# crockwell/far

Measured on AMD Instinct MI355X. Metric: image-pairs/sec (match+solve+regress) at 640x480, higher is better.
Workload: dtype f32

## Files before the change

### far_amd/_lib.py

```python
import ctypes
import os

from . import flags

_HERE = os.path.dirname(os.path.abspath(__file__))
LIB_PATH = flags.value('FAR_HIP_LIB') or os.path.join(_HERE, 'lib', 'libfar_hip.so')

c_p = ctypes.c_void_p
c_i = ctypes.c_int
c_f = ctypes.c_float
c_d = ctypes.c_double
c_sz = ctypes.c_size_t
c_l = ctypes.c_long
c_u32 = ctypes.c_uint32

SIGNATURES = {
    'far_abi_version': (c_i, []),
    'far_last_hip_error': (c_i, []),
    'far_set_tuning': (c_i, [c_i, c_i]),
    'far_mfma_probe_f16': (c_i, [c_i, c_i, c_i, c_p, c_p, c_p]),
    'far_dual_softmax_workspace_bytes': (c_sz, [c_i, c_i, c_i]),
    'far_dual_softmax_stats_f32': (c_i, [c_p, c_p, c_i, c_i, c_i, c_i, c_f, c_f, c_f, c_p, c_p, c_p, c_p, c_p, c_p]),
    'far_coarse_match_f32': (c_i, [c_p, c_p, c_i, c_i, c_i, c_i, c_f, c_f, c_i, c_i, c_i, c_i, c_i, c_f,
                                   c_p, c_p, c_p, c_p, c_p, c_p, c_p, c_p, c_p, c_p, c_p, c_p, c_p, c_p, c_p, c_p]),
    'far_coarse_match_bf16_workspace_bytes': (c_sz, [c_i, c_i, c_i, c_i]),
    'far_coarse_match_bf16': (c_i, [c_p, c_p, c_i, c_i, c_i, c_i, c_f, c_f, c_i, c_i, c_i, c_i, c_i, c_f,
                                    c_p, c_p, c_p, c_p, c_p, c_p, c_p, c_p, c_p, c_p, c_p, c_p, c_p, c_p, c_p, c_p]),
    'far_coarse_match_f16s_workspace_bytes': (c_sz, [c_i, c_i, c_i, c_i]),
    'far_coarse_match_f16s': (c_i, [c_p, c_p, c_i, c_i, c_i, c_i, c_f, c_f, c_i, c_i, c_i, c_i, c_i, c_f,
                                    c_p, c_p, c_p, c_p, c_p, c_p, c_p, c_p, c_p, c_p, c_p, c_p, c_p, c_p, c_p, c_p, c_p]),
    'far_conf_matrix_f16s': (c_i, [c_p, c_p, c_i, c_i, c_i, c_i, c_f, c_p, c_p, c_i, c_p, c_p, c_p, c_p, c_p]),
    'far_coarse_match_sinkhorn_f16s_workspace_bytes': (c_sz, [c_i, c_i, c_i, c_i]),
    'far_coarse_match_sinkhorn_f16s': (c_i, [c_p, c_p, c_i, c_i, c_i, c_i, c_p, c_i, c_i, c_f, c_i, c_i, c_i, c_i, c_i, c_f,
                                             c_p, c_p, c_p, c_p, c_p, c_p, c_p, c_p, c_p, c_p, c_p, c_p, c_p, c_p, c_p, c_p,
                                             c_p, c_p, c_p]),
    'far_coarse_train_workspace_bytes': (c_sz, [c_i, c_i, c_i, c_i]),
    'far_coarse_pos_conf_f16s': (c_i, [c_p, c_p, c_i, c_i, c_i, c_i, c_f, c_p, c_p, c_p, c_i, c_p, c_p, c_p, c_p]),
    'far_coarse_pos_conf_bwd_f16': (c_i, [c_p, c_p, c_i, c_i, c_i, c_i, c_f, c_p, c_p, c_p, c_i, c_p, c_p, c_p, c_p, c_p]),
    'far_sinkhorn_pos_conf_workspace_bytes': (c_sz, [c_i, c_i, c_i, c_i, c_i]),
    'far_sinkhorn_pos_conf_f16s': (c_i, [c_p, c_p, c_i, c_i, c_i, c_i, c_p, c_i, c_p, c_p, c_p, c_p, c_p, c_i, c_p, c_p, c_p,
                                         c_p, c_p, c_p]),
    'far_sinkhorn_pos_conf_bwd_f16': (c_i, [c_p, c_p, c_i, c_i, c_i, c_i, c_p, c_i, c_p, c_p, c_p, c_p, c_p, c_i, c_p, c_p, c_p,
                                            c_p, c_p, c_p, c_p, c_p]),
    'far_emm_pv_f32': (c_i, [c_p, c_p, c_p, c_p, c_i, c_i, c_i, c_f, c_p, c_p, c_p, c_p]),
    'far_fine_gather_f32': (c_i, [c_p, c_l, c_l, c_l, c_l, c_i, c_i, c_i, c_p, c_p, c_i, c_i, c_i, c_i, c_p, c_p]),
    'far_fine_scatter_f32': (c_i, [c_p, c_l, c_l, c_l, c_l, c_i, c_i, c_i, c_p, c_p, c_i, c_i, c_i, c_i, c_p, c_p]),
    'far_fine_scatter_det_f32': (c_i, [c_p, c_l, c_l, c_l, c_l, c_i, c_i, c_i, c_p, c_p, c_i, c_i, c_i, c_i, c_i, c_i, c_p, c_p]),
    'far_fine_expect_f32': (c_i, [c_p, c_p, c_i, c_i, c_i, c_p, c_f, c_p, c_p, c_p, c_p, c_p]),
    'far_linear_attention_workspace_bytes': (c_sz, [c_i, c_i, c_i, c_i]),
    'far_linear_attention_f32': (c_i, [c_p, c_p, c_p, c_i, c_i, c_i, c_i, c_i, c_p, c_p, c_f, c_p, c_p, c_p]),
    'far_linear_attention_apply_f32': (c_i, [c_p, c_p, c_i, c_i, c_i, c_i, c_p, c_f, c_p, c_p]),
    'far_full_attention_workspace_bytes': (c_sz, [c_i, c_i, c_i, c_i, c_i]),
    'far_full_attention_f16s': (c_i, [c_p, c_p, c_p, c_i, c_i, c_i, c_i, c_i, c_p, c_p, c_i, c_p, c_p, c_p, c_p]),
    'far_full_attention_train_f16s': (c_i, [c_p, c_p, c_p, c_i, c_i, c_i, c_i, c_i, c_p, c_p, c_i, c_p, c_p, c_p, c_p, c_p]),
    'far_full_attention_bwd_workspace_bytes': (c_sz, [c_i, c_i, c_i, c_i, c_i]),
    'far_full_attention_bwd_f16s': (c_i, [c_p, c_p, c_p, c_p, c_p, c_p, c_i, c_i, c_i, c_i, c_i, c_p, c_p, c_i, c_p, c_p, c_p, c_p, c_p, c_p]),
    'far_linear_attention_bwd_workspace_bytes': (c_sz, [c_i, c_i, c_i, c_i, c_i]),
    'far_linear_attention_bwd_f32': (c_i, [c_p, c_p, c_p, c_p, c_i, c_i, c_i, c_i, c_i, c_p, c_p, c_f, c_p, c_p, c_p, c_p, c_p]),
    'far_layernorm_f32': (c_i, [c_p, c_p, c_p, c_p, c_l, c_i, c_f, c_p, c_p]),
    'far_layernorm_bwd_ws_bytes': (c_l, [c_l, c_i]),
    'far_layernorm_bwd_f32': (c_i, [c_p, c_p, c_p, c_l, c_i, c_f, c_p, c_p, c_p, c_p, c_l, c_p]),
    'far_attn_block_packed_bytes': (c_sz, [c_i]),
    'far_attn_block_f16s': (c_i, [c_p, c_p, c_p, c_l, c_i, c_i, c_i, c_i, c_f, c_f, c_f, c_f, c_f, c_p, c_p, c_f, c_p, c_p, c_p]),
    'far_mlp_fused_packed_bytes': (c_sz, [c_i]),
    'far_mlp_fused_f16s': (c_i, [c_p, c_p, c_p, c_l, c_i, c_f, c_f, c_p, c_p, c_f, c_p, c_p, c_p]),
    'far_mlp_fused_f16': (c_i, [c_p, c_p, c_p, c_l, c_i, c_f, c_f, c_p, c_p, c_f, c_p, c_p, c_p]),
    'far_attn_block_f16': (c_i, [c_p, c_p, c_p, c_l, c_i, c_i, c_i, c_i, c_f, c_f, c_f, c_f, c_f, c_p, c_p, c_f, c_p, c_p, c_p]),
    'far_affine_act_f32': (c_i, [c_p, c_p, c_p, c_p, c_l, c_i, c_l, c_i, c_i, c_f, c_p, c_p]),
    'far_upsample2x_add_f32': (c_i, [c_p, c_p, c_i, c_i, c_i, c_i, c_i, c_p, c_p]),
    'far_upsample2x_bwd_f32': (c_i, [c_p, c_i, c_i, c_i, c_i, c_p, c_p]),
    'far_adamw_table_bytes': (c_l, [c_i, c_l]),
    'far_adamw_step_f32': (c_i, [c_p, c_i, c_l] + [ctypes.c_double] * 7 + [c_p]),
    'far_prior_from_pose_f32': (c_i, [c_p, c_p, c_p, c_i, c_p, c_p]),
    'far_bn_train_ws_bytes': (c_l, [c_l, c_i]),
    'far_bn_act_train_fwd_f32': (c_i, [c_p, c_p, c_l, c_i, c_p, c_p, c_f, c_f, c_p, c_p, c_i, c_f, c_p, c_p, c_p, c_l, c_p]),
    'far_bn_train_stats_f32': (c_i, [c_p, c_l, c_i, c_p, c_p, c_f, c_f, c_p, c_p, c_p, c_p, c_p, c_p, c_p, c_l, c_p]),
    'far_bn_train_bwd_f32': (c_i, [c_p, c_p, c_p, c_p, c_p, c_p, c_l, c_i, c_i, c_f, c_p, c_p, c_p, c_p, c_p, c_l, c_p]),
    'far_conv_packed_bytes': (c_sz, [c_i, c_i, c_i, c_i, c_i]),
    'far_conv_pack_f32': (c_i, [c_p, c_i, c_i, c_i, c_i, c_i, c_i, c_p, c_p]),
    'far_weight_scale_f32': (c_i, [c_p, c_l, c_p, c_p]),
    'far_conv_pack_view_f32': (c_i, [c_p, c_l, c_l, c_l, c_i, c_i, c_i, c_i, c_i, c_p, c_p, c_p]),
    'far_enc_layer_saved_floats': (c_l, [c_p]),
    'far_enc_layer_grads_floats': (c_l, [c_p]),
# ... 126 lines not shown
```

### far_amd/csrc/dual_softmax_f16s.hip

```cpp
#include "k1_f16s.h"
#include <algorithm>

int far_k1_conf_launch(const _Float16* ah, const _Float16* bh, int Z, int L, int S, int Lp, int Sp, float c1, float fill2,
                       const uint8_t* mask0, const uint8_t* mask1, const float2* rowstat, const float* cmax,
                       const float* cinv, float* conf, const int* fix_count, const uint2* fix_list, int slots,
                       int* fix_info_out, hipStream_t stream);

namespace {

constexpr int CAND_SLOTS = 4;

#define FAR_DPP(old, v, ctrl, rowmask) \
    __builtin_bit_cast(float, __builtin_amdgcn_update_dpp(__builtin_bit_cast(int, old), __builtin_bit_cast(int, v), ctrl, rowmask, 0xF, false))
__device__ __forceinline__ float max32_to_upper_row(float v) {
    v = fmaxf(v, FAR_DPP(v, v, 0xB1, 0xF));
    v = fmaxf(v, FAR_DPP(v, v, 0x4E, 0xF));
    v = fmaxf(v, FAR_DPP(v, v, 0x141, 0xF));
    v = fmaxf(v, FAR_DPP(v, v, 0x140, 0xF));
    v = fmaxf(v, FAR_DPP(v, v, 0x142, 0xA));
    return v;
}

template <bool CAND>
__global__ __launch_bounds__(256, 2) void k1_rowstats(const _Float16* __restrict__ ah, const _Float16* __restrict__ al,
// ... 42 lines not shown
        const float resc = __builtin_amdgcn_exp2f(m - mn);
        float t = 0.f;
#pragma unroll
        for (int ct = 0; ct < 2; ++ct)
#pragma unroll
            for (int r = 0; r < 16; ++r) t += __builtin_amdgcn_exp2f(acc[ct][r] - mn);
        sum *= resc;
        comp *= resc;
        const float y = t - comp;
        const float ns = sum + y;
        comp = (ns - sum) - y;
        sum = ns;
        m = mn;
        if (CAND) {
            const float clog = m + __builtin_amdgcn_logf(sum - comp);
            float hot = -1.f;
            const float* tl = reinterpret_cast<const float*>(lds + 2 * TILE_PLANE);
#pragma unroll
            for (int ct = 0; ct < 2; ++ct)
#pragma unroll
                for (int q4 = 0; q4 < 4; ++q4) {
                    const float4 a = *reinterpret_cast<const float4*>(tl + 32 * ct + 8 * q4 + 4 * h);
                    hot = fmaxf(hot, fmaxf(fmaxf(2.0f * acc[ct][4 * q4 + 0] - a.x, 2.0f * acc[ct][4 * q4 + 1] - a.y),
                                           fmaxf(2.0f * acc[ct][4 * q4 + 2] - a.z, 2.0f * acc[ct][4 * q4 + 3] - a.w)));
                }
            if (__builtin_amdgcn_ballot_w64(hot >= clog) != 0ull) {
                uint2* const slots = cand + ((size_t)z * Nr + min(irow, Nr - 1)) * (2 * CAND_SLOTS) + h * CAND_SLOTS;
#pragma unroll 1
                for (int ct = 0; ct < 2; ++ct)
#pragma unroll
                    for (int r = 0; r < 16; ++r) {
                        const int i = jt * KT + 32 * ct + mfma32_row(r, h);
                        const float xv = ct == 0 ? acc[0][r] : acc[1][r];
                        if (2.0f * xv >= tl[32 * ct + mfma32_row(r, h)] + clog && xv > -1.0e8f && i < Nc && irow < Nr) {
                            if (ncand < CAND_SLOTS) slots[ncand] = make_uint2((unsigned)i, __float_as_uint(xv));
                            ++ncand;
                        }
                    }
            }
        }
    }
    if (CAND && irow < Nr) cand_count[((size_t)z * Nr + irow) * 2 + h] = ncand;
    sum -= comp;
    const float mo = shfl_xor_f(m, 32), so = shfl_xor_f(sum, 32);
    const float mn = fmaxf(m, mo);
    const float st = sum * __builtin_amdgcn_exp2f(m - mn) + so * __builtin_amdgcn_exp2f(mo - mn);
    if (h == 0) {
        if (irow < Nr) stat[(size_t)z * Nr + irow] = make_float2(mn, st);
        if (dmax) {
            dmax[(size_t)z * Nrp + irow] = irow < Nr ? mn : HUGE_F;
            dinv[(size_t)z * Nrp + irow] = irow < Nr ? 1.0f / st : 0.f;
        }
        if (dthr) dthr[(size_t)z * Nrp + irow] = irow < Nr ? mn + __builtin_amdgcn_logf(st) - 12.0f : HUGE_F;
    }
}

__global__ __launch_bounds__(256, 2) void k1_screen(const _Float16* __restrict__ ah, const _Float16* __restrict__ bh, int Z, int L, int S,
                                                    int Lp, int Sp, float c1, const float2* __restrict__ rowstat,
                                                    const float* __restrict__ cmax, float thr, const unsigned* __restrict__ nmax,
                                                    uint8_t* __restrict__ tmask) {
    extern __shared__ __attribute__((aligned(16))) unsigned char lds[];
    const int tid = threadIdx.x, wave = tid >> 6, lane = tid & 63, l31 = lane & 31, h = lane >> 5;
    const int nI = Lp / 128;
    int z, Ib;
    tile_coords(nI, Z, z, Ib);
    const int irow = Ib * 128 + 32 * wave + l31;
    f16x8 rh[NS];
#pragma unroll
    for (int s = 0; s < NS; ++s)
        rh[s] = *reinterpret_cast<const f16x8*>(ah + ((size_t)z * Lp + irow) * C + 8 * ((2 * s + h) ^ (irow & 15)));
    const float rmax = irow < L ? rowstat[(size_t)z * L + irow].x : HUGE_F;
    const float c2 = 2.0f * c1;
    const float slack2 = c2 * __builtin_sqrtf(__uint_as_float(nmax[0]) * __uint_as_float(nmax[1])) *
                         (1.0f / 1024.0f * (1.0f + 1.0f / 2048.0f) + 1.0f / 8192.0f);
    const float lim = __builtin_amdgcn_logf(thr) + rmax - slack2;
    const int ntile = (S + KT - 1) / KT;
    for (int jt = 0; jt < ntile; ++jt) {
        __syncthreads();
        {
            const unsigned char* sh = reinterpret_cast<const unsigned char*>(bh + ((size_t)z * Sp + jt * KT) * C) + tid * 16;
#pragma unroll
            for (int j = 0; j < TILE_PLANE / 4096; ++j)
                __builtin_amdgcn_global_load_lds((gptr_t)(sh + j * 4096), (lptr_t)(lds + j * 4096 + wave * 1024), 16, 0, 0);
        }
        asm volatile("s_waitcnt vmcnt(0)" ::: "memory");
        __syncthreads();
        f32x16 acc[2];
#pragma unroll
        for (int ct = 0; ct < 2; ++ct)
#pragma unroll
            for (int r = 0; r < 16; ++r) acc[ct][r] = 0.f;
#pragma unroll
        for (int s = 0; s < NS; ++s)
#pragma unroll
            for (int ct = 0; ct < 2; ++ct) {
                const int row = 32 * ct + l31;
                const f16x8 ch = *reinterpret_cast<const f16x8*>(lds + row * ROWB + (((2 * s + h) ^ (row & 15)) * 16));
                acc[ct] = __builtin_amdgcn_mfma_f32_32x32x16_f16(ch, rh[s], acc[ct], 0, 0, 0);
            }
        float top = -HUGE_F;
#pragma unroll
        for (int ct = 0; ct < 2; ++ct)
#pragma unroll
            for (int q4 = 0; q4 < 4; ++q4) {
                const float4 a = *reinterpret_cast<const float4*>(cmax + (size_t)z * Sp + jt * KT + 32 * ct + 8 * q4 + 4 * h);
                top = fmaxf(top, fmaxf(fmaxf(fmaf(acc[ct][4 * q4 + 0], c2, -a.x), fmaf(acc[ct][4 * q4 + 1], c2, -a.y)),
// ... 49 lines not shown
                const size_t o = (size_t)z * Sp + jt * KT + 32 * ct + 8 * q4 + 4 * h;
                const float4 a = *reinterpret_cast<const float4*>(cmax + o), b = *reinterpret_cast<const float4*>(cinv + o);
                cm[4 * q4 + 0] = a.x; cm[4 * q4 + 1] = a.y; cm[4 * q4 + 2] = a.z; cm[4 * q4 + 3] = a.w;
                ci[4 * q4 + 0] = b.x; ci[4 * q4 + 1] = b.y; ci[4 * q4 + 2] = b.z; ci[4 * q4 + 3] = b.w;
            }
#pragma unroll
            for (int r = 0; r < 16; ++r) {
                const int j = jt * KT + 32 * ct + mfma32_row(r, h);
                float x2 = acc[ct][r] * c2;
                if (masks && j < S && (rmasked || (mask1 && !mask1[(size_t)z * S + j]))) x2 = 2.0f * fill2;
                const float p = __builtin_amdgcn_exp2f((x2 - rst.x) - cm[r]) * rinv * ci[r];
                const bool valid = ivalid && j < S;
                acc[ct][r] = valid ? p : -1.f;
                if (valid && p > bestv) { bestv = p; bestj = j; }
            }
            if (CONF && ivalid) {
#pragma unroll
                for (int q4 = 0; q4 < 4; ++q4) {
                    const int j = jt * KT + 32 * ct + 8 * q4 + 4 * h;
                    float* dst = conf + ((size_t)z * L + irow) * S + j;
                    if (aligned4 && j + 3 < S) {
                        *reinterpret_cast<float4*>(dst) = make_float4(acc[ct][4 * q4], acc[ct][4 * q4 + 1], acc[ct][4 * q4 + 2], acc[ct][4 * q4 + 3]);
                    } else {
#pragma unroll
                        for (int e = 0; e < 4; ++e)
                            if (j + e < S) dst[e] = acc[ct][4 * q4 + e];
                    }
                }
            }
            float tmax = fmaxf(fmaxf(acc[ct][0], acc[ct][1]), fmaxf(acc[ct][2], acc[ct][3]));
#pragma unroll
            for (int r = 4; r < 16; r += 2) tmax = fmaxf(tmax, fmaxf(acc[ct][r], acc[ct][r + 1]));
            if (__builtin_amdgcn_ballot_w64(tmax > thr) != 0ull) {
#pragma unroll
                for (int r = 0; r < 16; ++r)
                    if (acc[ct][r] > thr)
                        atomicMax(colbest + (size_t)z * S + jt * KT + 32 * ct + mfma32_row(r, h), __float_as_uint(acc[ct][r]));
            }
        }
    }
    const float vo = shfl_xor_f(bestv, 32);
    const int jo = shfl_xor_i(bestj, 32);
    if (vo > bestv || (vo == bestv && jo < bestj)) { bestv = vo; bestj = jo; }
    if (h == 0 && ivalid) {
        rowbest_v[(size_t)z * L + irow] = bestv;
        rowbest_j[(size_t)z * L + irow] = bestj;
    }
}

struct Ws16 {
    K1Workspace k;
    _Float16 *ah, *al, *bh, *bl;
    float2* colstat2;
    float *cmax, *cinv;
    float* rthr;
    uint8_t* tmask;
    unsigned* nmax;
    int* fix_count;
    uint2* fix_list;
    size_t bytes;
};
inline Ws16 carve16(void* ws, int Z, int L, int S) {
    Ws16 w;
    w.k = carve(ws, Z, L, S);
    const int Lp = (L + 127) / 128 * 128, Sp = (S + 127) / 128 * 128;
    unsigned char* p = (unsigned char*)ws;
    size_t o = w.k.bytes;
    auto take = [&](size_t n) { unsigned char* r = p ? p + o : nullptr; o += align256(n); return r; };
    w.ah = (_Float16*)take((size_t)Z * Lp * C * 2); w.al = (_Float16*)take((size_t)Z * Lp * C * 2);
    w.bh = (_Float16*)take((size_t)Z * Sp * C * 2); w.bl = (_Float16*)take((size_t)Z * Sp * C * 2);
    w.colstat2 = (float2*)take((size_t)Z * S * 8);
    w.cmax = (float*)take((size_t)Z * Sp * 4); w.cinv = (float*)take((size_t)Z * Sp * 4);
    w.rthr = (float*)take((size_t)Z * Lp * 4);
    w.nmax = (unsigned*)take(2 * sizeof(unsigned));
    w.tmask = (uint8_t*)take((size_t)Z * (Lp / 128) * ((S + KT - 1) / KT) * 4);
    w.fix_count = (int*)take((size_t)Z * S * 2 * sizeof(int));
    w.fix_list = (uint2*)take((size_t)Z * S * 2 * CAND_SLOTS * sizeof(uint2));
    w.bytes = o;
    return w;
}

}

size_t far_k1_fwd_ws_bytes(int Z, int L, int S) { return carve16(nullptr, Z, L, S).bytes; }

static float k1_c1(float temperature) {
    return (float)(1.4426950408889634 / ((double)C * (double)temperature * PRESCALE * PRESCALE));
}

int far_k1_stats_launch(const float* f0, const float* f1, int Z, int L, int S, float temperature, void* ws, int* overflow,
                        hipStream_t stream) {
    const Ws16 w = carve16(ws, Z, L, S);
    const int Lp = (L + 127) / 128 * 128, Sp = (S + 127) / 128 * 128;
    const float c1 = k1_c1(temperature), fill2 = -1e9f * 1.44269504088896341f;
    auto gridp = [](long n) { long b = (n + 255) / 256; return (unsigned)(b < 65536L * 4 ? b : 65536L * 4); };
    hipLaunchKernelGGL(k1_prep, dim3(gridp((long)Z * Lp * 32)), dim3(256), 0, stream, f0, Z, L, Lp, w.ah, w.al, overflow, (unsigned*)nullptr);
    hipLaunchKernelGGL(k1_prep, dim3(gridp((long)Z * Sp * 32)), dim3(256), 0, stream, f1, Z, S, Sp, w.bh, w.bl, overflow, (unsigned*)nullptr);
    const size_t smem_s = 2 * TILE_PLANE + KT * sizeof(float);
    FAR_ONCE_PER_DEVICE(hipFuncSetAttribute((const void*)k1_rowstats<false>, hipFuncAttributeMaxDynamicSharedMemorySize, (int)smem_s));
    hipLaunchKernelGGL(k1_rowstats<false>, dim3((Lp / 128) * Z), dim3(256), smem_s, stream, w.ah, w.al, w.bh, w.bl, Z, L, S, Lp, Sp,
                       c1, fill2, (const uint8_t*)nullptr, (const uint8_t*)nullptr, w.k.rowstat, (float*)nullptr, (float*)nullptr,
                       (float*)nullptr, (const float*)nullptr, (int*)nullptr, (uint2*)nullptr);
    hipLaunchKernelGGL(k1_rowstats<false>, dim3((Sp / 128) * Z), dim3(256), smem_s, stream, w.bh, w.bl, w.ah, w.al, Z, S, L, Sp, Lp,
                       c1, fill2, (const uint8_t*)nullptr, (const uint8_t*)nullptr, w.colstat2, w.cmax, w.cinv, (float*)nullptr,
                       (const float*)nullptr, (int*)nullptr, (uint2*)nullptr);
    return far_check_launch();
}

void far_k1_fwd_views(void* ws, int Z, int L, int S, const _Float16** ah, const _Float16** bh, const float2** rowstat,
                      const float** cmax, const float** cinv, float* c1_out) {
    const Ws16 w = carve16(ws, Z, L, S);
    *ah = w.ah; *bh = w.bh; *rowstat = w.k.rowstat; *cmax = w.cmax; *cinv = w.cinv;
    *c1_out = 0.f;
}

extern "C" {

size_t far_coarse_match_f16s_workspace_bytes(int Z, int L, int S, int Cc) {
    if (Z <= 0 || L <= 0 || S <= 0 || Cc != C) return 0;
    return carve16(nullptr, Z, L, S).bytes;
}

int far_coarse_match_f16s(const float* f0, const float* f1, int Z, int L, int S, int Cc,
                          float temperature, float thr, int border, int h0, int w0, int h1, int w1,
                          float cell_scale, const uint8_t* mask0, const uint8_t* mask1,
                          const int* valid_hw, const float* scale0, const float* scale1,
                          float* conf_out, int64_t* b_ids, int64_t* i_ids, int64_t* j_ids, float* mconf,
                          float* mkpts0_c, float* mkpts1_c, int* counts_out, int* total_out,
                          void* ws, int* overflow, hipStream_t stream) {
    far_clear_errors();
    if (!f0 || !f1 || !ws || !b_ids || !i_ids || !j_ids || !mconf || !mkpts0_c || !mkpts1_c || !total_out)
        return FAR_EINVAL;
    if (Z <= 0 || L <= 0 || S <= 0 || Cc != C || h0 * w0 != L || h1 * w1 != S || (long)Z * (L > S ? L : S) > 0x7ff00000L) return FAR_EINVAL;
    const Ws16 w = carve16(ws, Z, L, S);
    const int Lp = (L + 127) / 128 * 128, Sp = (S + 127) / 128 * 128;
    const float c1 = (float)(1.4426950408889634 / ((double)C * (double)temperature * PRESCALE * PRESCALE));
    const float fill2 = -1e9f * 1.44269504088896341f;
    auto gridp = [](long n) { long b = (n + 255) / 256; return (unsigned)(b < 65536L * 4 ? b : 65536L * 4); };
    const bool screen = !conf_out && !mask0 && !mask1 && far_get_tuning(10) == 0;
    if (screen) hipMemsetAsync(w.nmax, 0, 2 * sizeof(unsigned), stream);
    hipLaunchKernelGGL(k1_prep, dim3(gridp((long)Z * Lp * 32)), dim3(256), 0, stream, f0, Z, L, Lp, w.ah, w.al, overflow, screen ? w.nmax : (unsigned*)nullptr);
    hipLaunchKernelGGL(k1_prep, dim3(gridp((long)Z * Sp * 32)), dim3(256), 0, stream, f1, Z, S, Sp, w.bh, w.bl, overflow, screen ? w.nmax + 1 : (unsigned*)nullptr);
    int* counts = counts_out ? counts_out : w.k.counts;
    hipMemsetAsync(counts, 0, sizeof(int) * Z, stream);
    const size_t smem_s = 2 * TILE_PLANE + KT * sizeof(float), smem_m = 2 * TILE_PLANE + 4 * 64 * sizeof(float);
    FAR_ONCE_PER_DEVICE(
        hipFuncSetAttribute((const void*)k1_rowstats<false>, hipFuncAttributeMaxDynamicSharedMemorySize, (int)smem_s);
        hipFuncSetAttribute((const void*)k1_match<false>, hipFuncAttributeMaxDynamicSharedMemorySize, (int)smem_m);
        hipFuncSetAttribute((const void*)k1_match<true>, hipFuncAttributeMaxDynamicSharedMemorySize, (int)smem_m));
    hipLaunchKernelGGL(k1_rowstats<false>, dim3((Lp / 128) * Z), dim3(256), smem_s, stream, w.ah, w.al, w.bh, w.bl, Z, L, S, Lp, Sp,
                       c1, fill2, mask0, mask1, w.k.rowstat, (float*)nullptr, (float*)nullptr, (float*)nullptr,
                       (const float*)nullptr, (int*)nullptr, (uint2*)nullptr);
    hipLaunchKernelGGL(k1_rowstats<false>, dim3((Sp / 128) * Z), dim3(256), smem_s, stream, w.bh, w.bl, w.ah, w.al, Z, S, L, Sp, Lp,
                       c1, fill2, mask1, mask0, w.colstat2, w.cmax, w.cinv, (float*)nullptr, (const float*)nullptr,
                       (int*)nullptr, (uint2*)nullptr);
    const int nI = Lp / 128;
    hipMemsetAsync(w.k.colbest_part, 0, sizeof(float) * (size_t)Z * S, stream);
    if (screen) {
        FAR_ONCE_PER_DEVICE(hipFuncSetAttribute((const void*)k1_screen, hipFuncAttributeMaxDynamicSharedMemorySize, (int)TILE_PLANE));
        hipLaunchKernelGGL(k1_screen, dim3(nI * Z), dim3(256), TILE_PLANE, stream, w.ah, w.bh, Z, L, S, Lp, Sp, c1, w.k.rowstat, w.cmax, thr,
                           (const unsigned*)w.nmax, w.tmask);
    }
    if (conf_out)
        hipLaunchKernelGGL(k1_match<true>, dim3(nI * Z), dim3(256), smem_m, stream, w.ah, w.al, w.bh, w.bl, Z, L, S, Lp, Sp, c1,
                           fill2, mask0, mask1, w.k.rowstat, w.cmax, w.cinv, conf_out, w.k.rowbest_v, w.k.rowbest_j, reinterpret_cast<unsigned*>(w.k.colbest_part), thr,
                           screen ? (const uint8_t*)w.tmask : (const uint8_t*)nullptr);
    else
        hipLaunchKernelGGL(k1_match<false>, dim3(nI * Z), dim3(256), smem_m, stream, w.ah, w.al, w.bh, w.bl, Z, L, S, Lp, Sp, c1,
                           fill2, mask0, mask1, w.k.rowstat, w.cmax, w.cinv, conf_out, w.k.rowbest_v, w.k.rowbest_j, reinterpret_cast<unsigned*>(w.k.colbest_part), thr,
                           screen ? (const uint8_t*)w.tmask : (const uint8_t*)nullptr);
    hipLaunchKernelGGL(k_finalize, dim3((L + 255) / 256, Z), dim3(256), 0, stream, w.k.rowbest_v, w.k.rowbest_j,
                       w.k.colbest_part, 1, L, S, thr, border, h0, w0, h1, w1, valid_hw, w.k.match_j, counts);
    hipLaunchKernelGGL(k_compact, dim3(Z), dim3(256), 0, stream, w.k.match_j, w.k.rowbest_v, counts, L, w0, w1,
                       cell_scale, scale0, scale1, b_ids, i_ids, j_ids, mconf, mkpts0_c, mkpts1_c, total_out);
    return far_check_launch();
}

int far_conf_matrix_f16s(const float* f0, const float* f1, int Z, int L, int S, int Cc, float temperature,
                         const uint8_t* mask0, const uint8_t* mask1, int stages, float* conf_out, int* fix_info_out,
                         void* ws, int* overflow, hipStream_t stream) {
    far_clear_errors();
    if (!f0 || !f1 || !ws || !conf_out || Z <= 0 || L <= 0 || S <= 0 || Cc != C || !(stages & 3) || (long)Z * (L > S ? L : S) > 0x7ff00000L) return FAR_EINVAL;
    const Ws16 w = carve16(ws, Z, L, S);
    const int Lp = (L + 127) / 128 * 128, Sp = (S + 127) / 128 * 128;
    const float c1 = (float)(1.4426950408889634 / ((double)C * (double)temperature * PRESCALE * PRESCALE));
    const float fill2 = -1e9f * 1.44269504088896341f;
    if (stages & 1) {
        auto gridp = [](long n) { long b = (n + 255) / 256; return (unsigned)(b < 65536L * 4 ? b : 65536L * 4); };
        hipLaunchKernelGGL(k1_prep, dim3(gridp((long)Z * Lp * 32)), dim3(256), 0, stream, f0, Z, L, Lp, w.ah, w.al, overflow, (unsigned*)nullptr);
        hipLaunchKernelGGL(k1_prep, dim3(gridp((long)Z * Sp * 32)), dim3(256), 0, stream, f1, Z, S, Sp, w.bh, w.bl, overflow, (unsigned*)nullptr);
        const size_t smem_s = 2 * TILE_PLANE + KT * sizeof(float);
        FAR_ONCE_PER_DEVICE(
            hipFuncSetAttribute((const void*)k1_rowstats<false>, hipFuncAttributeMaxDynamicSharedMemorySize, (int)smem_s);
            hipFuncSetAttribute((const void*)k1_rowstats<true>, hipFuncAttributeMaxDynamicSharedMemorySize, (int)smem_s));
        hipLaunchKernelGGL(k1_rowstats<false>, dim3((Lp / 128) * Z), dim3(256), smem_s, stream, w.ah, w.al, w.bh, w.bl, Z, L, S, Lp,
                           Sp, c1, fill2, mask0, mask1, w.k.rowstat, (float*)nullptr, (float*)nullptr, w.rthr,
                           (const float*)nullptr, (int*)nullptr, (uint2*)nullptr);
        hipLaunchKernelGGL(k1_rowstats<true>, dim3((Sp / 128) * Z), dim3(256), smem_s, stream, w.bh, w.bl, w.ah, w.al, Z, S, L, Sp,
                           Lp, c1, fill2, mask1, mask0, w.colstat2, w.cmax, w.cinv, (float*)nullptr, (const float*)w.rthr,
                           w.fix_count, w.fix_list);
    }
    if (stages & 2) {
        const int rc = far_k1_conf_launch(w.ah, w.bh, Z, L, S, Lp, Sp, c1, fill2, mask0, mask1, w.k.rowstat, w.cmax, w.cinv,
                                          conf_out, w.fix_count, w.fix_list, CAND_SLOTS, fix_info_out, stream);
        if (rc != FAR_OK) return rc;
    }
    return far_check_launch();
}

}
```

### far_amd/flags.py

```python
import os
from collections import namedtuple

Switch = namedtuple('Switch', 'env module attr off_value neutral scope doc')
SWITCHES = [
    Switch('FAR_NO_WINO', 'far_amd.ops', 'USE_WINO', False, 'parity', 'inference',
           'stride-1 3x3 convolutions on K9 (direct implicit GEMM) instead of K17 (Winograd F(2x2,3x3)); same operator, other summation'),
    Switch('FAR_NO_PAD', 'far_amd.loftr.backbone', 'PAD_CHANNELS', False, 'bitwise', 'inference',
           'the 196-channel backbone maps stored with 196 channels instead of 208 (zero weights for the extra ones: exact zeros)'),
    Switch('FAR_NO_PREFETCH', 'far_amd.loftr.model:LoFTR', 'head_prefetch', False, 'bitwise', 'inference',
           "the head's feature stage computed inside forward_rt_prediction instead of enqueued behind K1"),
    Switch('FAR_NO_SIDE_STREAM', 'far_amd.loftr.model:LoFTR', 'head_side_stream', False, 'bitwise', 'inference',
           "the head's feature stage on the step's own stream behind K1 (rounds 2-5) instead of on a second stream next to K1 and the fine level"),
    Switch('FAR_FPN_STREAM', 'far_amd.loftr.model:LoFTR', 'fpn_side_stream', True, 'bitwise', 'inference',
           "OPT-IN (1 switches it ON; default off): the FPN's fine branch on a side stream next to the coarse transformer and K1 (-0.6 ms per 32 "
           "pairs; off by default because the roofline launch -- K17 208 -> 208 @ 240x320 -- then shares the GPU and its in-step duration "
           "in a kernel trace is no longer its own)"),
    Switch('FAR_NO_GATHER_FUSE', 'far_amd.loftr.stages:FinePreprocess', 'fused_gather', False, 'bitwise', 'inference',
           'FinePreprocess.merge_feat on a materialised window tensor (K3 gather + K9) instead of K9 reading through the match indices'),
    Switch('FAR_NO_KV', 'far_amd.loftr.transformer:LoFTREncoderLayer', 'fused_kv', False, 'parity', 'inference',
           "k, v projections + K5's first half as separate launches instead of K9's k|v epilogue (the K'^T V sum changes order)"),
    Switch('FAR_NO_QAPPLY', 'far_amd.loftr.transformer:LoFTREncoderLayer', 'fused_apply', False, 'parity', 'inference',
           "q projection + K5's second half as separate launches instead of K9's attention-apply epilogue (q no longer stays in split operands)"),
    Switch('FAR_NO_STACK', 'far_amd.loftr.transformer:LocalFeatureTransformer', 'stack_self', False, 'bitwise', 'inference',
           "the two 'self' calls of an encoder layer on the two images separately instead of one call on both"),
    Switch('FAR_NO_BN', 'far_amd.ops', 'USE_HIP_BATCHNORM_TRAIN', False, 'parity', 'training',
           'training-mode BatchNorm on nn.BatchNorm2d + torch activations instead of K19 (tests/test_train_kernels_gpu.py holds K19 to the module)'),
]

ENV_ONLY = {
    'FAR_HIP_LIB': ('load', 'path of another build of libfar_hip.so (tools/ab_build.py: same-box A/B against a git revision); skips the build-id check'),
    'FAR_TUNING': ('load', 'comma-separated key=value pairs handed to far_set_tuning at load time, e.g. FAR_TUNING="10=1,8=1" (keys below)'),
    'FAR_SKIP_ASM_CHECK': ('build', "1: far_amd/build.py does not scan the generated code (K9's asm pixel loads; the LDS-DMA ring rule of every kernel with global_load_lds; the half-register writes of the asm fp16 split) after recompiling"),
    'FAR_EXTRA_HIPCC_FLAGS': ('build', 'extra hipcc flags of an experiment build (-DFAR_WINO_EXP=..., tools/wino_exp.sh); part of the build id'),
    'FAR_COMMIT': ('tools', 'commit stamp tools/collect_profiles.sh / tools/step_floors.py write into the profile files'),
    'FAR_C3_PY_NODE': ('bench', "bench.py --workload c3: the encoder layer's autograd node driven from Python instead of far_enc_layer_fwd / _bwd"),
    'FAR_C3_NO_OVERLAP': ('bench', 'bench.py --workload c3: the layer node without side streams'),
    'FAR_C3_PER_OP': ('bench', 'bench.py --workload c3: one autograd node per operator instead of per layer'),
    'FAR_TORCH_ADAMW': ('bench', 'bench.py --workload c3: torch.optim.AdamW instead of K20'),
    'FAR_CUDNN_BENCHMARK': ('bench', 'bench.py: torch.backends.cudnn.benchmark for the vendor comparison legs'),
}

Tuning = namedtuple('Tuning', 'key default values neutral doc')
TUNING = [
    Tuning(0, 3, (0, 1, 2, 4, 7), 'bitwise', 'bit mask of exact-f32 kernels that stagger wave-slot priorities: 1 k_stats, 2 k_match, 4 k_emm_pv'),
    Tuning(1, 0, (1,), 'parity', 'K1 exact-f32 variant: the other tile shape (another summation order of the row statistics)'),
    Tuning(2, 0, (1,), 'bitwise', 'conf_matrix writer variant A (store pattern)'),
    Tuning(3, 0, (1,), 'bitwise', 'conf_matrix writer variant B (store pattern)'),
    Tuning(4, 0, (1,), 'bitwise', 'K9 without the seven-tile mode / K5 windows on the generic path'),
    Tuning(5, 0, (1, 2, 4), 'bitwise', 'K5 apply: tiles per unit'),
    Tuning(6, 0, (64, 256), 'parity', "K5: tokens per K'^T V chunk (another partial-sum grouping)"),
    Tuning(7, 0, (1,), 'bitwise', 'K9 Linear launches always on full-height tiles'),
    Tuning(8, 0, (1,), 'bitwise', 'K17 splits its operands with the five-instruction split2 instead of v_fma_mix (same values)'),
    Tuning(9, 0, (1,), 'bitwise', 'K17 runs a short last channel block on the full body'),
    Tuning(10, 0, (1,), 'bitwise', "K1's match pass without the tile prescreen"),
    Tuning(11, 0, (1, 2), 'bitwise', "K14's pipeline: 0 = 4 waves / 3 slots / counted waits, two workgroups per CU; 1 = 8 waves / 4 slots / counted, one per CU (round 5's form); 2 = 4 waves / 3 slots / vmcnt(0) per phase (fallback without a wait table)"),
    Tuning(12, 0, (1,), 'parity', "K10's inference form on the exact-f32 matrix instruction instead of split fp16"),
    Tuning(15, 0, (1,), 'bitwise', 'K17: 1 = the multiplying wave group does NOT raise its issue priority (the round-4 kernel)'),
    Tuning(13, 0, (1,), 'bitwise', "K9's FPN-merge epilogue in its generic form everywhere"),
]


def off(env):
    if env not in {s.env for s in SWITCHES}:
        raise KeyError(f'{env} is not a registered far_amd switch (far_amd/flags.py)')
    return os.environ.get(env, '0') not in ('', '0')


def value(env, default=None):
    if env not in ENV_ONLY:
        raise KeyError(f'{env} is not a registered far_amd environment variable (far_amd/flags.py)')
    return os.environ.get(env, default)


def known():
    return {s.env for s in SWITCHES} | set(ENV_ONLY)


def unknown_in_environment():
    skip = ('FAR_WINO_', 'FAR_K9_')
    return sorted(k for k in os.environ if k.startswith('FAR_') and k not in known() and not k.startswith(skip))


def target(sw):
    import importlib
    mod, _, cls = sw.module.partition(':')
    obj = importlib.import_module(mod)
    return (getattr(obj, cls) if cls else obj), sw.attr
```

### include/far_hip.h

```cpp
#ifndef FAR_HIP_H
#define FAR_HIP_H

#include <stddef.h>
#include <stdint.h>

#ifdef __cplusplus
extern "C" {
#endif

typedef struct ihipStream_t* far_stream_t;

int far_abi_version(void);
const char* far_build_id(void);
int far_last_hip_error(void);
int far_set_tuning(int key, int value);

void* far_stream_fork(far_stream_t main, int i);
int far_stream_join(far_stream_t main, int i);

int far_mfma_probe_f16(int mode, int iters, int rounds, float* sink, double* flops_out, far_stream_t stream);


size_t far_dual_softmax_workspace_bytes(int Z, int L, int S);

int far_dual_softmax_stats_f32(const float* f0, const float* f1, int Z, int L, int S, int C,
                               float feat_div, float sim_div, float sim_mul,
                               const uint8_t* mask0, const uint8_t* mask1,
                               float* rowstat_out, float* colstat_out, void* ws, far_stream_t stream);

int far_coarse_match_f32(const float* f0, const float* f1, int Z, int L, int S, int C,
                         float temperature, float thr, int border, int h0, int w0, int h1, int w1,
                         float cell_scale, const uint8_t* mask0, const uint8_t* mask1,
                         const int* valid_hw, const float* scale0, const float* scale1,
                         float* conf_out, int64_t* b_ids, int64_t* i_ids, int64_t* j_ids, float* mconf,
                         float* mkpts0_c, float* mkpts1_c, int* counts_out, int* total_out,
                         void* ws, far_stream_t stream);

size_t far_coarse_match_bf16_workspace_bytes(int Z, int L, int S, int C);
int far_coarse_match_bf16(const float* f0, const float* f1, int Z, int L, int S, int C,
                          float temperature, float thr, int border, int h0, int w0, int h1, int w1,
                          float cell_scale, const uint8_t* mask0, const uint8_t* mask1,
                          const int* valid_hw, const float* scale0, const float* scale1,
                          float* conf_out, int64_t* b_ids, int64_t* i_ids, int64_t* j_ids, float* mconf,
                          float* mkpts0_c, float* mkpts1_c, int* counts_out, int* total_out,
                          void* ws, far_stream_t stream);

size_t far_coarse_match_f16s_workspace_bytes(int Z, int L, int S, int C);
int far_coarse_match_f16s(const float* f0, const float* f1, int Z, int L, int S, int C,
                          float temperature, float thr, int border, int h0, int w0, int h1, int w1,
                          float cell_scale, const uint8_t* mask0, const uint8_t* mask1,
                          const int* valid_hw, const float* scale0, const float* scale1,
                          float* conf_out, int64_t* b_ids, int64_t* i_ids, int64_t* j_ids, float* mconf,
                          float* mkpts0_c, float* mkpts1_c, int* counts_out, int* total_out,
                          void* ws, int* overflow, far_stream_t stream);

int far_conf_matrix_f16s(const float* f0, const float* f1, int Z, int L, int S, int C, float temperature,
                         const uint8_t* mask0, const uint8_t* mask1, int stages, float* conf_out, int* fix_info_out,
                         void* ws, int* overflow, far_stream_t stream);

size_t far_coarse_match_sinkhorn_f16s_workspace_bytes(int Z, int L, int S, int C);
int far_coarse_match_sinkhorn_f16s(const float* f0, const float* f1, int Z, int L, int S, int C,
                                   const float* bin_score, int iters, int prefilter, float thr, int border,
                                   int h0, int w0, int h1, int w1, float cell_scale, const uint8_t* mask0, const uint8_t* mask1,
                                   const int* valid_hw, const float* scale0, const float* scale1,
                                   float* conf_with_bin, float* log_u, float* log_v,
                                   int64_t* b_ids, int64_t* i_ids, int64_t* j_ids, float* mconf,
                                   float* mkpts0_c, float* mkpts1_c, int* counts_out, int* total_out,
                                   void* ws, int* overflow, far_stream_t stream);

size_t far_coarse_train_workspace_bytes(int Z, int L, int S, int C);
int far_coarse_pos_conf_f16s(const float* f0, const float* f1, int Z, int L, int S, int C, float temperature,
                             const int64_t* pb, const int64_t* pi, const int64_t* pj, int M, float* p_out, void* ws,
                             int* overflow, far_stream_t stream);
int far_coarse_pos_conf_bwd_f16(const float* f0, const float* f1, int Z, int L, int S, int C, float temperature,
                                const int64_t* pb, const int64_t* pi, const int64_t* pj, int M, const float* w,
                                float* df0, float* df1, void* ws, far_stream_t stream);

size_t far_sinkhorn_pos_conf_workspace_bytes(int Z, int L, int S, int C, int iters);
int far_sinkhorn_pos_conf_f16s(const float* f0, const float* f1, int Z, int L, int S, int C, const float* bin_score, int iters,
                               const uint8_t* mask0, const uint8_t* mask1, const int64_t* pb, const int64_t* pi, const int64_t* pj,
                               int M, float* conf_pos, float* conf_bin0, float* conf_bin1, void* ws, int* overflow,
                               far_stream_t stream);
int far_sinkhorn_pos_conf_bwd_f16(const float* f0, const float* f1, int Z, int L, int S, int C, const float* bin_score, int iters,
                                  const uint8_t* mask0, const uint8_t* mask1, const int64_t* pb, const int64_t* pi, const int64_t* pj,
                                  int M, const float* w_pos, const float* w_bin0, const float* w_bin1, float* df0, float* df1,
                                  float* dbin, void* ws, far_stream_t stream);


int far_emm_pv_f32(const float* q, const float* k, const float* v, const float* pos, int Z, int N, int D,
                   float scale, const float* rowstat, const float* colstat, float* T_out, far_stream_t stream);

size_t far_emm_pv_f16s_workspace_bytes(int Z, int N);
int far_emm_pv_f16s(const float* q, const float* k, const float* v, const float* pos, int Z, int N, int D, float scale,
                    int heads, long head_stride, long prob_stride, int q_rot, void* ws, float* T_out, int* overflow,
                    far_stream_t stream);
int far_emm_pv_f16(const float* q, const float* k, const float* v, const float* pos, int Z, int N, int D, float scale,
                   int heads, long head_stride, long prob_stride, int q_rot, void* ws, float* T_out, int* overflow,
                   far_stream_t stream);
int far_emm_pv_f16s_copy_stats(const void* ws, int Z, int N, float* rowstat_out, float* colstat_out, far_stream_t stream);

size_t far_emm_bwd_workspace_bytes(int Z, int N);
int far_emm_bwd_f16(const float* q, const float* k, const float* vt, const float* A, const float* u, const float* vw,
                    const float* rowstat, const float* colstat, int Z, int N, float scale, float* dq, float* dk,
                    void* ws, far_stream_t stream);


int far_fine_gather_f32(const float* feat, long sn, long sc, long sh, long sw, int C, int Hf, int Wf,
// ... 225 lines not shown
```

Before: 378.7.

## Fuse row and column softmax statistics into one score pass with column reduce

Replaces the two k1_rowstats launches, which each recompute the full score matrix for row and for column stats, with a single k1_stats2 kernel. It computes each score tile once, keeps running row stats and writes per-32-row column partial max/sum through an LDS transpose. A new k1_colreduce kernel merges the partials into column stats. This halves the MFMA score work in the dual-softmax stats phase, at the cost of a partial buffer, extra LDS and a changed column summation order. The fused path is used for unmasked calls by default, and a screen-view query helper is also exported.

```diff
diff --git a/far_amd/_lib.py b/far_amd/_lib.py
--- a/far_amd/_lib.py
+++ b/far_amd/_lib.py
@@ -29,6 +29,7 @@
     'far_coarse_match_f16s_workspace_bytes': (c_sz, [c_i, c_i, c_i, c_i]),
     'far_coarse_match_f16s': (c_i, [c_p, c_p, c_i, c_i, c_i, c_i, c_f, c_f, c_i, c_i, c_i, c_i, c_i, c_f,
                                     c_p, c_p, c_p, c_p, c_p, c_p, c_p, c_p, c_p, c_p, c_p, c_p, c_p, c_p, c_p, c_p, c_p]),
+    'far_coarse_match_f16s_screen_view': (c_i, [c_i, c_i, c_i, c_p, c_p]),
     'far_conf_matrix_f16s': (c_i, [c_p, c_p, c_i, c_i, c_i, c_i, c_f, c_p, c_p, c_i, c_p, c_p, c_p, c_p, c_p]),
     'far_coarse_match_sinkhorn_f16s_workspace_bytes': (c_sz, [c_i, c_i, c_i, c_i]),
     'far_coarse_match_sinkhorn_f16s': (c_i, [c_p, c_p, c_i, c_i, c_i, c_i, c_p, c_i, c_i, c_f, c_i, c_i, c_i, c_i, c_i, c_f,
diff --git a/far_amd/csrc/dual_softmax_f16s.hip b/far_amd/csrc/dual_softmax_f16s.hip
--- a/far_amd/csrc/dual_softmax_f16s.hip
+++ b/far_amd/csrc/dual_softmax_f16s.hip
@@ -118,6 +118,124 @@
             dinv[(size_t)z * Nrp + irow] = irow < Nr ? 1.0f / st : 0.f;
         }
         if (dthr) dthr[(size_t)z * Nrp + irow] = irow < Nr ? mn + __builtin_amdgcn_logf(st) - 12.0f : HUGE_F;
+    }
+}
+
+constexpr int TR_BYTES = 32 * 32 * 4;
+__global__ __launch_bounds__(256, 2) void k1_stats2(const _Float16* __restrict__ ah, const _Float16* __restrict__ al,
+                                                    const _Float16* __restrict__ bh, const _Float16* __restrict__ bl,
+                                                    int Z, int Nr, int Nc, int Nrp, int Ncp, float c1,
+                                                    float2* __restrict__ stat, float2* __restrict__ colpart) {
+    extern __shared__ __attribute__((aligned(16))) unsigned char lds[];
+    const int tid = threadIdx.x, wave = tid >> 6, lane = tid & 63, l31 = lane & 31, h = lane >> 5;
+    int z, Ib;
+    tile_coords(Nrp / 128, Z, z, Ib);
+    const int irow = Ib * 128 + 32 * wave + l31;
+    RowFrags rf;
+    rf.load(ah, al, (size_t)z * Nrp + irow, irow, h);
+    float* const tr = reinterpret_cast<float*>(lds + 2 * TILE_PLANE + wave * TR_BYTES);
+    const bool padrows = Ib * 128 + 32 * wave + 31 >= Nr;
+    const bool rvalid = irow < Nr;
+    const int wq = l31 >> 2, wr = l31 & 3;
+    const float* const rd = tr + l31 * 32;
+    const int rsw = (l31 >> 1) & 7;
+    float2* const cp = colpart + ((size_t)z * (Nrp / 32) + Ib * 4 + wave) * Ncp + l31;
+    float m = -HUGE_F, sum = 0.f, comp = 0.f;
+    const int ntile = (Nc + KT - 1) / KT;
+    for (int jt = 0; jt < ntile; ++jt) {
+        __syncthreads();
+        dma_tile(lds, bh, bl, (size_t)z * Ncp + jt * KT, tid, wave);
+        asm volatile("s_waitcnt vmcnt(0)" ::: "memory");
+        __syncthreads();
+        f32x16 acc[2];
+        score_tile(acc, lds, rf, l31, h);
+        const bool special = (jt + 1) * KT > Nc;
+        float tm = -HUGE_F;
+#pragma unroll
+        for (int ct = 0; ct < 2; ++ct)
+#pragma unroll
+            for (int r = 0; r < 16; ++r) {
+                float x = acc[ct][r] * c1;
+                if (special && jt * KT + 32 * ct + mfma32_row(r, h) >= Nc) x = -HUGE_F;
+                acc[ct][r] = x;
+                tm = fmaxf(tm, x);
+            }
+#pragma unroll
+        for (int ct = 0; ct < 2; ++ct) {
+            asm volatile("" ::: "memory");
+#pragma unroll
+            for (int r = 0; r < 16; ++r) {
+                const int c = mfma32_row(r, h);
+                float x = acc[ct][r];
+                if (padrows && !rvalid) x = -HUGE_F;
+                tr[c * 32 + ((wq ^ ((c >> 1) & 7)) << 2) + wr] = x;
+            }
+            asm volatile("" ::: "memory");
+            float4 v[4];
+#pragma unroll
+            for (int k = 0; k < 4; ++k) v[k] = *reinterpret_cast<const float4*>(rd + (((4 * h + k) ^ rsw) << 2));
+            float cm = fmaxf(fmaxf(v[0].x, v[0].y), fmaxf(v[0].z, v[0].w));
+#pragma unroll
+            for (int k = 1; k < 4; ++k) cm = fmaxf(cm, fmaxf(fmaxf(v[k].x, v[k].y), fmaxf(v[k].z, v[k].w)));
+            float cs = 0.f;
+#pragma unroll
+            for (int k = 0; k < 4; ++k)
+                cs += (__builtin_amdgcn_exp2f(v[k].x - cm) + __builtin_amdgcn_exp2f(v[k].y - cm)) +
+                      (__builtin_amdgcn_exp2f(v[k].z - cm) + __builtin_amdgcn_exp2f(v[k].w - cm));
+            const float mo = shfl_xor_f(cm, 32), so = shfl_xor_f(cs, 32);
+            const float cmn = fmaxf(cm, mo);
+            const float cst = cs * __builtin_amdgcn_exp2f(cm - cmn) + so * __builtin_amdgcn_exp2f(mo - cmn);
+            if (h == 0) cp[jt * KT + 32 * ct] = make_float2(cmn, cst);
+        }
+        const float mn = fmaxf(m, tm);
+        const float resc = __builtin_amdgcn_exp2f(m - mn);
+        float t = 0.f;
+#pragma unroll
+        for (int ct = 0; ct < 2; ++ct)
+#pragma unroll
+            for (int r = 0; r < 16; ++r) t += __builtin_amdgcn_exp2f(acc[ct][r] - mn);
+        sum *= resc;
+        comp *= resc;
+        const float y = t - comp;
+        const float ns = sum + y;
+        comp = (ns - sum) - y;
+        sum = ns;
+        m = mn;
+    }
+    sum -= comp;
+    const float mo = shfl_xor_f(m, 32), so = shfl_xor_f(sum, 32);
+    const float mn = fmaxf(m, mo);
+    const float st = sum * __builtin_amdgcn_exp2f(m - mn) + so * __builtin_amdgcn_exp2f(mo - mn);
+    if (h == 0 && irow < Nr) stat[(size_t)z * Nr + irow] = make_float2(mn, st);
+}
+
+__global__ __launch_bounds__(256) void k1_colreduce(const float2* __restrict__ colpart, int L, int S, int Sp, int nG,
+                                                    float2* __restrict__ colstat2, float* __restrict__ cmax, float* __restrict__ cinv) {
+    __shared__ float smax[4][64];
+    __shared__ double ssum[4][64];
+    const int c = threadIdx.x & 63, seg = threadIdx.x >> 6;
+    const int nJ = Sp / 64, z = blockIdx.x / nJ, j = (blockIdx.x - z * nJ) * 64 + c;
+    const int ng = (L + 31) / 32;
+    const float2* const p = colpart + (size_t)z * nG * Sp + j;
+    float mx = -HUGE_F;
+#pragma unroll 4
+    for (int g = seg; g < ng; g += 4) mx = fmaxf(mx, p[(size_t)g * Sp].x);
+    smax[seg][c] = mx;
+    __syncthreads();
+    mx = fmaxf(fmaxf(smax[0][c], smax[1][c]), fmaxf(smax[2][c], smax[3][c]));
+    double s = 0.0;
+#pragma unroll 4
+    for (int g = seg; g < ng; g += 4) {
+        const float2 q = p[(size_t)g * Sp];
+        s += (double)q.y * (double)__builtin_amdgcn_exp2f(q.x - mx);
+    }
+    ssum[seg][c] = s;
+    __syncthreads();
+    if (seg == 0) {
+        const float st = (float)(((ssum[0][c] + ssum[1][c]) + ssum[2][c]) + ssum[3][c]);
+        if (j < S) colstat2[(size_t)z * S + j] = make_float2(mx, st);
+        cmax[(size_t)z * Sp + j] = j < S ? mx : HUGE_F;
+        cinv[(size_t)z * Sp + j] = j < S ? 1.0f / st : 0.f;
     }
 }
 
@@ -273,6 +391,7 @@
     K1Workspace k;
     _Float16 *ah, *al, *bh, *bl;
     float2* colstat2;
+    float2* colpart;
     float *cmax, *cinv;
     float* rthr;
     uint8_t* tmask;
@@ -297,6 +416,7 @@
     w.tmask = (uint8_t*)take((size_t)Z * (Lp / 128) * ((S + KT - 1) / KT) * 4);
     w.fix_count = (int*)take((size_t)Z * S * 2 * sizeof(int));
     w.fix_list = (uint2*)take((size_t)Z * S * 2 * CAND_SLOTS * sizeof(uint2));
+    w.colpart = (float2*)take((size_t)Z * (Lp / 32) * Sp * sizeof(float2));
     w.bytes = o;
     return w;
 }
@@ -359,6 +479,7 @@
     const float fill2 = -1e9f * 1.44269504088896341f;
     auto gridp = [](long n) { long b = (n + 255) / 256; return (unsigned)(b < 65536L * 4 ? b : 65536L * 4); };
     const bool screen = !conf_out && !mask0 && !mask1 && far_get_tuning(10) == 0;
+    const bool fused = !mask0 && !mask1 && far_get_tuning(14) == 0;
     if (screen) hipMemsetAsync(w.nmax, 0, 2 * sizeof(unsigned), stream);
     hipLaunchKernelGGL(k1_prep, dim3(gridp((long)Z * Lp * 32)), dim3(256), 0, stream, f0, Z, L, Lp, w.ah, w.al, overflow, screen ? w.nmax : (unsigned*)nullptr);
     hipLaunchKernelGGL(k1_prep, dim3(gridp((long)Z * Sp * 32)), dim3(256), 0, stream, f1, Z, S, Sp, w.bh, w.bl, overflow, screen ? w.nmax + 1 : (unsigned*)nullptr);
@@ -369,12 +490,21 @@
         hipFuncSetAttribute((const void*)k1_rowstats<false>, hipFuncAttributeMaxDynamicSharedMemorySize, (int)smem_s);
         hipFuncSetAttribute((const void*)k1_match<false>, hipFuncAttributeMaxDynamicSharedMemorySize, (int)smem_m);
         hipFuncSetAttribute((const void*)k1_match<true>, hipFuncAttributeMaxDynamicSharedMemorySize, (int)smem_m));
-    hipLaunchKernelGGL(k1_rowstats<false>, dim3((Lp / 128) * Z), dim3(256), smem_s, stream, w.ah, w.al, w.bh, w.bl, Z, L, S, Lp, Sp,
-                       c1, fill2, mask0, mask1, w.k.rowstat, (float*)nullptr, (float*)nullptr, (float*)nullptr,
-                       (const float*)nullptr, (int*)nullptr, (uint2*)nullptr);
-    hipLaunchKernelGGL(k1_rowstats<false>, dim3((Sp / 128) * Z), dim3(256), smem_s, stream, w.bh, w.bl, w.ah, w.al, Z, S, L, Sp, Lp,
-                       c1, fill2, mask1, mask0, w.colstat2, w.cmax, w.cinv, (float*)nullptr, (const float*)nullptr,
-                       (int*)nullptr, (uint2*)nullptr);
+    if (fused) {
+        const size_t smem_f = 2 * TILE_PLANE + 4 * TR_BYTES;
+        FAR_ONCE_PER_DEVICE(hipFuncSetAttribute((const void*)k1_stats2, hipFuncAttributeMaxDynamicSharedMemorySize, (int)smem_f));
+        hipLaunchKernelGGL(k1_stats2, dim3((Lp / 128) * Z), dim3(256), smem_f, stream, w.ah, w.al, w.bh, w.bl, Z, L, S, Lp, Sp, c1,
+                           w.k.rowstat, w.colpart);
+        hipLaunchKernelGGL(k1_colreduce, dim3((Sp / 64) * Z), dim3(256), 0, stream, (const float2*)w.colpart, L, S, Sp, Lp / 32,
+                           w.colstat2, w.cmax, w.cinv);
+    } else {
+        hipLaunchKernelGGL(k1_rowstats<false>, dim3((Lp / 128) * Z), dim3(256), smem_s, stream, w.ah, w.al, w.bh, w.bl, Z, L, S, Lp, Sp,
+                           c1, fill2, mask0, mask1, w.k.rowstat, (float*)nullptr, (float*)nullptr, (float*)nullptr,
+                           (const float*)nullptr, (int*)nullptr, (uint2*)nullptr);
+        hipLaunchKernelGGL(k1_rowstats<false>, dim3((Sp / 128) * Z), dim3(256), smem_s, stream, w.bh, w.bl, w.ah, w.al, Z, S, L, Sp, Lp,
+                           c1, fill2, mask1, mask0, w.colstat2, w.cmax, w.cinv, (float*)nullptr, (const float*)nullptr,
+                           (int*)nullptr, (uint2*)nullptr);
+    }
     const int nI = Lp / 128;
     hipMemsetAsync(w.k.colbest_part, 0, sizeof(float) * (size_t)Z * S, stream);
     if (screen) {
@@ -395,6 +525,15 @@
     hipLaunchKernelGGL(k_compact, dim3(Z), dim3(256), 0, stream, w.k.match_j, w.k.rowbest_v, counts, L, w0, w1,
                        cell_scale, scale0, scale1, b_ids, i_ids, j_ids, mconf, mkpts0_c, mkpts1_c, total_out);
     return far_check_launch();
+}
+
+int far_coarse_match_f16s_screen_view(int Z, int L, int S, size_t* offset, size_t* bytes) {
+    if (Z <= 0 || L <= 0 || S <= 0 || !offset || !bytes) return FAR_EINVAL;
+    const uintptr_t base = 256;
+    const Ws16 w = carve16(reinterpret_cast<void*>(base), Z, L, S);
+    *offset = (size_t)(reinterpret_cast<uintptr_t>(w.tmask) - base);
+    *bytes = (size_t)Z * ((L + 127) / 128) * ((S + KT - 1) / KT) * 4;
+    return FAR_OK;
 }
 
 int far_conf_matrix_f16s(const float* f0, const float* f1, int Z, int L, int S, int Cc, float temperature,
diff --git a/far_amd/flags.py b/far_amd/flags.py
--- a/far_amd/flags.py
+++ b/far_amd/flags.py
@@ -57,6 +57,7 @@
     Tuning(12, 0, (1,), 'parity', "K10's inference form on the exact-f32 matrix instruction instead of split fp16"),
     Tuning(15, 0, (1,), 'bitwise', 'K17: 1 = the multiplying wave group does NOT raise its issue priority (the round-4 kernel)'),
     Tuning(13, 0, (1,), 'bitwise', "K9's FPN-merge epilogue in its generic form everywhere"),
+    Tuning(14, 0, (1,), 'parity', "K1 split-fp16, unmasked calls: both softmax statistics on two k1_rowstats launches instead of k1_stats2 + k1_colreduce (the column sums change their summation order)"),
 ]
 
 
diff --git a/include/far_hip.h b/include/far_hip.h
--- a/include/far_hip.h
+++ b/include/far_hip.h
@@ -53,6 +53,7 @@
                           float* conf_out, int64_t* b_ids, int64_t* i_ids, int64_t* j_ids, float* mconf,
                           float* mkpts0_c, float* mkpts1_c, int* counts_out, int* total_out,
                           void* ws, int* overflow, far_stream_t stream);
+int far_coarse_match_f16s_screen_view(int Z, int L, int S, size_t* offset, size_t* bytes);
 
 int far_conf_matrix_f16s(const float* f0, const float* f1, int Z, int L, int S, int C, float temperature,
                          const uint8_t* mask0, const uint8_t* mask1, int stages, float* conf_out, int* fix_info_out,
```

Result: no change. 382.3, median of 6 (+1.0%).
